# zhengyk19/vit-rpe-rope

Hardware: AMD Instinct MI355X
Metric: train images/sec, CIFAR-10 ViT d=192 L=6 H=6 (higher is better)
Workload: dtype bf16; 1 GPU; CIFAR-10-shaped 32x32 patch4 ViT d=192 L=6 H=6, --pos_encoding rope-axial theta=100, bf16, full train step (fwd+CE+bwd+AdamW), random-init weights; per_gpu_batch=512, global_batch=512, parallelism=dp1, hip_graph=True

## Files before the change

vit-rpe-rope_amd/csrc/misc.hip:

```cpp
#include "common.h"
#include "augment.h"

namespace vitpe {

template <typename T>
__global__ void unfold_kernel(const float* __restrict__ img, T* __restrict__ patches, int B, int Cc, int S, int p) {
  const int g = S / p, P = g * g, Kp = Cc * p * p;
  const long long total = (long long)B * P * Cc * p;
  for (long long idx = (long long)blockIdx.x * blockDim.x + threadIdx.x; idx < total;
       idx += (long long)gridDim.x * blockDim.x) {
    const int ky = (int)(idx % p);
    long long t = idx / p;
    const int ch = (int)(t % Cc); t /= Cc;
    const int n = (int)(t % P);
    const int b = (int)(t / P);
    const int gy = n / g, gx = n % g;
    const float* src = img + (((size_t)b * Cc + ch) * S + gy * p + ky) * S + gx * p;
    T* dst = patches + ((size_t)b * P + n) * Kp + ch * p * p + ky * p;
    for (int kx = 0; kx < p; ++kx) dst[kx] = from_f32<T>(src[kx]);
  }
}

__global__ void unfold8_kernel(const float* __restrict__ img, bf16* __restrict__ patches, int B, int Cc, int S, int p) {
  const int g = S / p, P = g * g, Kp = Cc * p * p, p8 = p / 8;
// ... 365 lines not shown
}

template <typename T, int KD, bool WLDS>
__global__ __launch_bounds__(256) void head_step_kernel(const T* __restrict__ x, const float* __restrict__ gamma,
                                                        const float* __restrict__ beta, const float* __restrict__ Wh,
                                                        const float* __restrict__ bh, const long long* __restrict__ labels,
                                                        float* __restrict__ logits, float* __restrict__ dlogits,
                                                        float* __restrict__ ws_xhat, float* __restrict__ ws_yn,
                                                        float* __restrict__ ws_dyn, T* __restrict__ dx,
                                                        float* __restrict__ per_image, const float* __restrict__ ctl,
                                                        int B, int Ntok, int D, int Cn, float eps) {
  constexpr int HS_LDS = 16 * 768;
  __shared__ float sWh[WLDS ? HS_LDS : 4];
  const int lane = threadIdx.x & 63, wave = threadIdx.x >> 6;
  const int b_raw = blockIdx.x * 4 + wave;
  const bool live = b_raw < B;
  const int b = live ? b_raw : B - 1;
  const float invD = 1.0f / (float)D;
  const float gscale = ctl[0], lscale = ctl[1];
  const int nvalid = min(B, (int)ctl[2]);
  const T* row = x + (size_t)b * Ntok * D;
  float xv[KD], gam[KD], bet[KD];
  float s = 0.f;
#pragma unroll
  for (int k = 0; k < KD; ++k) {
    const int d = lane + 64 * k;
    const bool ok = d < D;
    xv[k] = ok ? to_f32(row[d]) : 0.f;
    gam[k] = ok ? gamma[d] : 0.f;
    bet[k] = ok ? beta[d] : 0.f;
  }
  if (WLDS)
    for (int i = threadIdx.x; i < Cn * D; i += 256) sWh[i] = Wh[i];
  __syncthreads();
  if (!live) return;
#pragma unroll
  for (int k = 0; k < KD; ++k) s += xv[k];
  const float mean = wave_sum(s) * invD;
  float s2 = 0.f;
#pragma unroll
  for (int k = 0; k < KD; ++k) { const float t = (lane + 64 * k < D) ? xv[k] - mean : 0.f; s2 += t * t; }
  const float rstd = 1.0f / sqrtf(wave_sum(s2) * invD + eps);
  float xh[KD], yn[KD];
#pragma unroll
  for (int k = 0; k < KD; ++k) {
    const int d = lane + 64 * k;
    xh[k] = (d < D) ? (xv[k] - mean) * rstd : 0.f;
    yn[k] = xh[k] * gam[k] + bet[k];
    if (d < D) { ws_xhat[(size_t)b * D + d] = xh[k]; ws_yn[(size_t)b * D + d] = yn[k]; }
  }
  float z = -3.0e38f;
  for (int c0 = 0; c0 < Cn; c0 += 8) {
    float part[8];
#pragma unroll
    for (int j = 0; j < 8; ++j) {
      part[j] = 0.f;
      const int cI = min(c0 + j, Cn - 1);
#pragma unroll
      for (int k = 0; k < KD; ++k) {
        const int d = lane + 64 * k;
        part[j] += (d < D) ? yn[k] * (WLDS ? sWh[cI * D + d] : Wh[(size_t)cI * D + d]) : 0.f;
      }
    }
#pragma unroll
    for (int o = 32; o >= 1; o >>= 1)
#pragma unroll
      for (int j = 0; j < 8; ++j) part[j] += __shfl_xor(part[j], o, 64);
#pragma unroll
    for (int j = 0; j < 8; ++j)
      if (lane == c0 + j && c0 + j < Cn) z = part[j] + bh[c0 + j];
  }
  if (lane < Cn) logits[(size_t)b * Cn + lane] = z;
  float m = z;
#pragma unroll
  for (int o = 32; o >= 1; o >>= 1) m = fmaxf(m, __shfl_xor(m, o, 64));
  int am = (lane < Cn && z == m) ? lane : 1 << 20;
#pragma unroll
  for (int o = 32; o >= 1; o >>= 1) am = min(am, __shfl_xor(am, o, 64));
  const float e = lane < Cn ? expf(z - m) : 0.f;
  const float se = wave_sum(e);
  const int y = (int)labels[b];
  const float zy = __shfl(z, y, 64);
  const bool valid = b < nvalid;
  const float dl = (lane < Cn && valid) ? (e * (1.0f / se) - (lane == y ? 1.f : 0.f)) * gscale : 0.f;
  if (lane < Cn) dlogits[(size_t)b * Cn + lane] = dl;
  float dyn[KD];
#pragma unroll
  for (int k = 0; k < KD; ++k) dyn[k] = 0.f;
  for (int c = 0; c < Cn; ++c) {
    const float dc = __shfl(dl, c, 64);
#pragma unroll
    for (int k = 0; k < KD; ++k) {
      const int d = lane + 64 * k;
      dyn[k] += (d < D) ? dc * (WLDS ? sWh[c * D + d] : Wh[(size_t)c * D + d]) : 0.f;
    }
  }
  float t1 = 0.f, t2 = 0.f;
#pragma unroll
  for (int k = 0; k < KD; ++k) {
    const int d = lane + 64 * k;
    if (d < D) ws_dyn[(size_t)b * D + d] = dyn[k];
    const float gv = dyn[k] * gam[k];
    t1 += gv;
    t2 += gv * xh[k];
  }
  t1 = wave_sum(t1) * invD;
  t2 = wave_sum(t2) * invD;
  T* drow = dx + (size_t)b * Ntok * D;
#pragma unroll
  for (int k = 0; k < KD; ++k) {
    const int d = lane + 64 * k;
    if (d < D) drow[d] = from_f32<T>(rstd * (dyn[k] * gam[k] - t1 - xh[k] * t2));
  }
  if (lane == 0) {
    per_image[2 * b] = valid ? ((m + logf(se)) - zy) * lscale : 0.f;
    per_image[2 * b + 1] = (valid && am == y) ? 1.f : 0.f;
  }
}

template <typename T>
__global__ __launch_bounds__(256) void head_bwd_rows_kernel(const float* __restrict__ dlogits, const float* __restrict__ Wh,
                                                            const float* __restrict__ gamma, const float* __restrict__ ws_xhat,
                                                            const float* __restrict__ ws_rstd, float* __restrict__ ws_dyn,
                                                            T* __restrict__ dx, int B, int Ntok, int D, int Cn) {
  const int lane = threadIdx.x & 63, wave = threadIdx.x >> 6;
  const float invD = 1.0f / (float)D;
  for (int b = blockIdx.x * 4 + wave; b < B; b += gridDim.x * 4) {
    float s1 = 0.f, s2 = 0.f;
    for (int d = lane; d < D; d += 64) {
      float dyn = 0.f;
      for (int k = 0; k < Cn; ++k) dyn += dlogits[(size_t)b * Cn + k] * Wh[(size_t)k * D + d];
      ws_dyn[(size_t)b * D + d] = dyn;
      const float gv = dyn * gamma[d];
      s1 += gv;
      s2 += gv * ws_xhat[(size_t)b * D + d];
    }
    s1 = wave_sum(s1) * invD;
    s2 = wave_sum(s2) * invD;
    const float rstd = ws_rstd[b];
    T* drow = dx + (size_t)b * Ntok * D;
    for (int d = lane; d < D; d += 64) {
      const float gv = ws_dyn[(size_t)b * D + d] * gamma[d];
      drow[d] = from_f32<T>(rstd * (gv - s1 - ws_xhat[(size_t)b * D + d] * s2));
    }
    if (D % CH<T>::n == 0) {
      const Chunk16 z16 = {0u, 0u, 0u, 0u};
      for (size_t q = D / CH<T>::n + lane; q < (size_t)Ntok * D / CH<T>::n; q += 64)
        *reinterpret_cast<Chunk16*>(drow + q * CH<T>::n) = z16;
    } else {
      for (size_t q = D + lane; q < (size_t)Ntok * D; q += 64) drow[q] = from_f32<T>(0.f);
    }
  }
}
__global__ void head_bwd_params_kernel(const float* __restrict__ dlogits, const float* __restrict__ ws_yn,
                                       const float* __restrict__ ws_dyn, const float* __restrict__ ws_xhat,
                                       float* dWh, float* dbh, float* dgamma, float* dbeta, int B, int D, int Cn,
                                       int bchunk, const float* __restrict__ per_image, float* out2, float* metric_acc,
                                       float* hp_tick) {
  if (hp_tick != nullptr && blockIdx.x == 0 && blockIdx.y == 0 && threadIdx.x == 0) {
    const float step = hp_tick[5] + 1.0f;
    hp_tick[5] = step;
    hp_tick[6] = 1.0f - powf(hp_tick[1], step);
    hp_tick[7] = 1.0f - powf(hp_tick[2], step);
  }
  if (per_image != nullptr && blockIdx.x == 0 && blockIdx.y == 0) {
    __shared__ float sl[256], sc[256];
    float l = 0.f, cr = 0.f;
    for (int b = threadIdx.x; b < B; b += 256) { l += per_image[2 * b]; cr += per_image[2 * b + 1]; }
    sl[threadIdx.x] = l;
    sc[threadIdx.x] = cr;
    __syncthreads();
    for (int o = 128; o >= 1; o >>= 1) {
      if (threadIdx.x < o) { sl[threadIdx.x] += sl[threadIdx.x + o]; sc[threadIdx.x] += sc[threadIdx.x + o]; }
      __syncthreads();
    }
    if (threadIdx.x == 0) {
      out2[0] = sl[0]; out2[1] = sc[0];
      if (metric_acc != nullptr) { metric_acc[0] += sl[0]; metric_acc[1] += sc[0]; }
    }
  }
  const int idx = blockIdx.x * blockDim.x + threadIdx.x;
  const int b0 = blockIdx.y * bchunk, b1 = min(B, b0 + bchunk);
  const int nW = Cn * D;
  if (idx < nW) {
    const int k = idx / D, d = idx % D;
    float s = 0.f;
    for (int b = b0; b < b1; ++b) s += dlogits[(size_t)b * Cn + k] * ws_yn[(size_t)b * D + d];
    atomicAdd(dWh + idx, s);
  } else if (idx < nW + Cn) {
    const int k = idx - nW;
    float s = 0.f;
    for (int b = b0; b < b1; ++b) s += dlogits[(size_t)b * Cn + k];
    atomicAdd(dbh + k, s);
  } else if (idx < nW + Cn + D) {
    const int d = idx - nW - Cn;
    float sg = 0.f, sb = 0.f;
    for (int b = b0; b < b1; ++b) {
      const float dy = ws_dyn[(size_t)b * D + d];
      sg += dy * ws_xhat[(size_t)b * D + d];
      sb += dy;
    }
    atomicAdd(dgamma + d, sg);
    atomicAdd(dbeta + d, sb);
  }
}

template <typename T>
__global__ void embed_bwd_kernel(const T* __restrict__ dtok, float* dcls, float* dape, T* __restrict__ dpatch,
                                 int B, int Ntok, int D, int bchunk) {
  const int idx = blockIdx.x * blockDim.x + threadIdx.x;
  if (idx >= Ntok * D) return;
  const int n = idx / D, d = idx % D;
  const int b0 = blockIdx.y * bchunk, b1 = min(B, b0 + bchunk);
  float s = 0.f;
  for (int b = b0; b < b1; ++b) {
    const T v = dtok[((size_t)b * Ntok + n) * D + d];
    s += to_f32(v);
    if (n >= 1) dpatch[((size_t)b * (Ntok - 1) + n - 1) * D + d] = v;
  }
  if (n == 0) atomicAdd(dcls + d, s);
  else if (dape) atomicAdd(dape + (size_t)(n - 1) * D + d, s);
}

__global__ void adamw_tick_kernel(float* hp) {
  const float step = hp[5] + 1.0f;
  hp[5] = step;
  hp[6] = 1.0f - powf(hp[1], step);
  hp[7] = 1.0f - powf(hp[2], step);
}
template <int GS>
__global__ void adamw_kernel(float* __restrict__ p, float* __restrict__ g, float* __restrict__ m, float* __restrict__ v,
                             bf16* __restrict__ shadow, const float* __restrict__ hp, long long n, int zero_grad) {
  const float lr = hp[0], b1 = hp[1], b2 = hp[2], eps = hp[3], wd = hp[4], bc1 = hp[6], bc2 = hp[7], gs = hp[GS];
  const float inv_sqrt_bc2 = 1.0f / sqrtf(bc2), step_size = lr / bc1;
  for (long long i = (long long)blockIdx.x * blockDim.x + threadIdx.x; i < n; i += (long long)gridDim.x * blockDim.x) {
    const float gi = g[i] * gs;
    float pi = p[i] * (1.0f - lr * wd);
    const float mi = b1 * m[i] + (1.0f - b1) * gi;
    const float vi = b2 * v[i] + (1.0f - b2) * gi * gi;
    pi -= step_size * mi / (sqrtf(vi) * inv_sqrt_bc2 + eps);
    p[i] = pi; m[i] = mi; v[i] = vi;
    if (shadow) shadow[i] = (bf16)pi;
    if (zero_grad) g[i] = 0.f;
  }
}

static inline int grad_clip_blocks(long long n) { return (int)min((n + 4095) / 4096, (long long)1024); }

__global__ __launch_bounds__(256) void grad_sqnorm_kernel(const float* __restrict__ g, long long n,
                                                          float* __restrict__ partial) {
  const long long head = min(n, (long long)((4 - (int)(((unsigned long long)g >> 2) & 3)) & 3));
  const float4* __restrict__ body = reinterpret_cast<const float4*>(g + head);
  const long long nvec = (n - head) >> 2;
  const long long stride = (long long)gridDim.x * 256;
  float c0 = 0.f, c1 = 0.f, c2 = 0.f, c3 = 0.f;
#define VITPE_SQ_ACC(q) do { c0 = fmaf(q.x, q.x, c0); c1 = fmaf(q.y, q.y, c1); c2 = fmaf(q.z, q.z, c2); c3 = fmaf(q.w, q.w, c3); } while (0)
  long long i = (long long)blockIdx.x * 256 + threadIdx.x;
  for (; i + 3 * stride < nvec; i += 4 * stride) {
    const float4 q0 = body[i], q1 = body[i + stride], q2 = body[i + 2 * stride], q3 = body[i + 3 * stride];
    VITPE_SQ_ACC(q0); VITPE_SQ_ACC(q1); VITPE_SQ_ACC(q2); VITPE_SQ_ACC(q3);
  }
  for (; i < nvec; i += stride) {
    const float4 q = body[i];
    VITPE_SQ_ACC(q);
  }
#undef VITPE_SQ_ACC
  if (blockIdx.x == 0) {
    const long long tail0 = head + 4 * nvec;
    const int t = threadIdx.x;
    if (t < head) c0 = fmaf(g[t], g[t], c0);
    if (t >= 64 && tail0 + (t - 64) < n) c0 = fmaf(g[tail0 + (t - 64)], g[tail0 + (t - 64)], c0);
  }
  float s = (c0 + c1) + (c2 + c3);
#pragma unroll
  for (int o = 32; o >= 1; o >>= 1) s += __shfl_xor(s, o, 64);
  __shared__ float ws[4];
  if ((threadIdx.x & 63) == 0) ws[threadIdx.x >> 6] = s;
  __syncthreads();
  if (threadIdx.x == 0) partial[blockIdx.x] = (ws[0] + ws[1]) + (ws[2] + ws[3]);
}
__global__ __launch_bounds__(64) void grad_clip_finalize_kernel(const float* __restrict__ partial, int nb, float* hp) {
  double s = 0.0;
  for (int i = threadIdx.x; i < nb; i += 64) s += (double)partial[i];
#pragma unroll
  for (int o = 32; o >= 1; o >>= 1) s += __shfl_xor(s, o, 64);
  if (threadIdx.x == 0) {
    const float gs = hp[8];
    const float norm = (float)((double)gs * sqrt(s));
    double coef = (double)hp[12] / ((double)norm + 1e-6);
    coef = coef > 1.0 ? 1.0 : coef;
    const float cf = nb == 0 ? 1.0f : (float)coef;
    hp[10] = norm;
    hp[11] = cf;
    hp[9] = gs * cf;
  }
}
template <typename T>
__global__ void cast_kernel(const float* __restrict__ src, T* __restrict__ dst, long long n) {
  for (long long i = (long long)blockIdx.x * blockDim.x + threadIdx.x; i < n; i += (long long)gridDim.x * blockDim.x)
    dst[i] = from_f32<T>(src[i]);
}
template <typename T>
__global__ void transpose_cast_kernel(const float* __restrict__ src, T* __restrict__ dst, int R, int Cc) {
  __shared__ float tile[32][33];
  const int r0 = blockIdx.y * 32, c0 = blockIdx.x * 32;
  for (int i = threadIdx.y; i < 32; i += 8) {
    const int r = r0 + i, c = c0 + threadIdx.x;
    tile[i][threadIdx.x] = (r < R && c < Cc) ? src[(size_t)r * Cc + c] : 0.f;
  }
  __syncthreads();
  for (int i = threadIdx.y; i < 32; i += 8) {
    const int c = c0 + i, r = r0 + threadIdx.x;
    if (c < Cc && r < R) dst[(size_t)c * R + r] = from_f32<T>(tile[threadIdx.x][i]);
  }
}

struct ShadowDesc { long long src_off, dst_off, dst_off2; int R, C, tile0, kind, HD, kind2, HD2, pad; };

template <typename T>
__global__ __launch_bounds__(256) void refresh_shadows_kernel(const float* __restrict__ flat, T* __restrict__ dst_base,
                                                              const ShadowDesc* __restrict__ desc, int ndesc,
                                                              const unsigned short* __restrict__ tile_map) {
  __shared__ float tile[32][33];
  int d = 0;
  if (tile_map != nullptr) {
    d = tile_map[blockIdx.x];
  } else {
    for (int i = 1; i < ndesc; ++i)
      if ((int)blockIdx.x >= desc[i].tile0) d = i;
  }
  const ShadowDesc ds = desc[d];
  const int t = blockIdx.x - ds.tile0;
  const int tc = (ds.C + 31) / 32;
  const int r0 = (t / tc) * 32, c0 = (t % tc) * 32;
  const float* src = flat + ds.src_off;
  const int tx = threadIdx.x & 31, ty = threadIdx.x >> 5;
  for (int i = ty; i < 32; i += 8) {
    const int r = r0 + i, c = c0 + tx;
    tile[i][tx] = (r < ds.R && c < ds.C) ? src[(size_t)r * ds.C + c] : 0.f;
  }
  __syncthreads();
  auto emit = [&](int kind, T* dst, int hd) {
    if (kind == 0) {
      for (int i = ty; i < 32; i += 8) {
        const int c = c0 + i, r = r0 + tx;
        if (c < ds.C && r < ds.R) dst[(size_t)c * ds.R + r] = from_f32<T>(tile[tx][i]);
      }
    } else if (kind == 6) {
      const int D = ds.C, S = D / 16;
      const float qs = 1.4426950408889634f * rsqrtf((float)hd);
      for (int i = ty; i < 32; i += 8) {
        const int r = r0 + i, c = c0 + tx;
        if (r < ds.R && c < ds.C) {
          const int mat = r / D, rr = r % D, h = rr / 32, f = rr % 32;
          const int sidx = c / 16, hh = (c % 16) / 8, e = c % 8;
          const size_t blk = ((size_t)(h * 3 + mat) * S + sidx);
          dst[(blk * 64 + f + 32 * hh) * 8 + e] = from_f32<T>(tile[i][tx] * (mat == 0 ? qs : 1.0f));
        }
      }
    } else if (kind >= 2) {
      const bool tr = kind >= 4, phi = (kind & 1) != 0;
      const int PR = tr ? ds.C : ds.R;
      const int p0 = tr ? c0 : r0, k0 = tr ? r0 : c0;
      const int kch = hd, KSC = kch / 32, NTr = PR / 16;
      const int kc = k0 / kch, ks = (k0 % kch) / 32;
      const int dd = threadIdx.x * 4, frag = dd >> 9, within = dd & 511, l = within >> 3, e0 = within & 7;
      const int nt = p0 / 16 + frag, cc = l & 15, g = l >> 4;
      if (16 * nt < PR) {
        float v[4];
#pragma unroll
        for (int j = 0; j < 4; ++j) {
          const int e = e0 + j;
          const int k = phi ? (e < 4 ? 4 * g + e : 16 + 4 * g + e - 4) : 8 * g + e;
          v[j] = tr ? tile[k][16 * frag + cc] : tile[16 * frag + cc][k];
        }
        const size_t blk = ((size_t)kc * NTr + nt) * KSC + ks;
        st4(dst + blk * 512 + within, v[0], v[1], v[2], v[3]);
      }
    } else {
      const int D = ds.C, HD = hd, NT = HD / 16, KS = D / 32;
      for (int i = ty; i < 32; i += 8) {
        const int r = r0 + i, c = c0 + tx;
        if (r < ds.R && c < ds.C) {
          const int mat = r / D, rr = r % D, h = rr / HD, nt = (rr % HD) / 16, cc = rr % 16;
          const int ks = c / 32, g = (c % 32) / 8, e = c % 8;
          const size_t blk = (((size_t)(h * 3 + mat) * NT + nt) * KS + ks);
          dst[(blk * 64 + 16 * g + cc) * 8 + e] = from_f32<T>(tile[i][tx]);
        }
      }
    }
  };
  emit(ds.kind, dst_base + ds.dst_off, ds.HD);
  if (ds.kind2 >= 0) emit(ds.kind2, dst_base + ds.dst_off2, ds.HD2);
}

template <typename T>
__global__ void selftest_mma_kernel(const T* __restrict__ A, const T* __restrict__ Bt, const T* __restrict__ Brow,
                                    float* __restrict__ C_row, float* __restrict__ C_tr) {
  __shared__ __attribute__((aligned(16))) T sB[32 * 24];
  const int lane = threadIdx.x, c = lane & 15, g = lane >> 4;
  for (int q = lane; q < 32 * 16; q += 64) sB[(q / 16) * 24 + (q % 16)] = Brow[q];
  __syncthreads();
  f32x4 acc = {0.f, 0.f, 0.f, 0.f};
  mma(ld_frag(A + c * 32 + 8 * g), ld_frag(Bt + c * 32 + 8 * g), acc);
  for (int r = 0; r < 4; ++r) C_row[(4 * g + r) * 16 + c] = acc[r];
  f32x4 acc2 = {0.f, 0.f, 0.f, 0.f};
  mma(ld_frag(A + c * 32 + 8 * g), ld_frag_tr(sB, 24, 8 * g, 8 * g + 4, 0), acc2);
  for (int r = 0; r < 4; ++r) C_tr[(4 * g + r) * 16 + c] = acc2[r];
}

}

using namespace vitpe;

#define GRID1D(n) dim3((unsigned)(((n) + 255) / 256)), dim3(256)

extern "C" int vitpe_unfold(int dtype, const float* img, void* patches, int B, int C, int S, int p, hipStream_t st) {
  VITPE_REQUIRE(img && patches && B >= 0 && C > 0 && p > 0 && S % p == 0 && (dtype == 0 || dtype == 1));
  const long long total = (long long)B * (S / p) * (S / p) * C * p;
  if (total == 0) return 0;
  const unsigned blocks = (unsigned)min((total + 255) / 256, (long long)8192);
  if (dtype == 1 && p % 8 == 0) {
    const long long total8 = total * (p / 8);
    hipLaunchKernelGGL(unfold8_kernel, dim3((unsigned)min((total8 + 255) / 256, (long long)16384)), dim3(256), 0, st, img,
                       (bf16*)patches, B, C, S, p);
    VITPE_CHECK_LAUNCH();
  }
  if (dtype == 1) hipLaunchKernelGGL(unfold_kernel<bf16>, dim3(blocks), dim3(256), 0, st, img, (bf16*)patches, B, C, S, p);
  else hipLaunchKernelGGL(unfold_kernel<float>, dim3(blocks), dim3(256), 0, st, img, (float*)patches, B, C, S, p);
  VITPE_CHECK_LAUNCH();
}

static int launch_unfold_u8(int dtype, const unsigned char* data, const long long* index, const float* mean,
                            const float* stdv, void* patches, float* img_out, int B, int C, int S, int p,
                            const unsigned long long* rng, int pad, int hflip, hipStream_t st) {
  VITPE_REQUIRE(data && mean && stdv && patches && B >= 0 && C > 0 && p > 0 && S % p == 0 && (dtype == 0 || dtype == 1));
  VITPE_REQUIRE(rng == nullptr || (pad >= 0 && pad <= S));
  const long long total = (long long)B * (S / p) * (S / p) * C * p;
  if (total == 0) return 0;
  const unsigned blocks = (unsigned)min((total + 255) / 256, (long long)8192);
  if (rng != nullptr) {
    if (dtype == 1)
      hipLaunchKernelGGL((unfold_u8_kernel<bf16, true>), dim3(blocks), dim3(256), 0, st, data, index, mean, stdv, (bf16*)patches, img_out, B, C, S, p, rng, pad, hflip);
    else
      hipLaunchKernelGGL((unfold_u8_kernel<float, true>), dim3(blocks), dim3(256), 0, st, data, index, mean, stdv, (float*)patches, img_out, B, C, S, p, rng, pad, hflip);
  } else {
    if (dtype == 1)
      hipLaunchKernelGGL((unfold_u8_kernel<bf16, false>), dim3(blocks), dim3(256), 0, st, data, index, mean, stdv, (bf16*)patches, img_out, B, C, S, p, rng, 0, 0);
    else
      hipLaunchKernelGGL((unfold_u8_kernel<float, false>), dim3(blocks), dim3(256), 0, st, data, index, mean, stdv, (float*)patches, img_out, B, C, S, p, rng, 0, 0);
  }
  VITPE_CHECK_LAUNCH();
}

extern "C" int vitpe_unfold_u8(int dtype, const unsigned char* data, const long long* index, const float* mean,
                               const float* stdv, void* patches, float* img_out, int B, int C, int S, int p,
                               hipStream_t st) {
  return launch_unfold_u8(dtype, data, index, mean, stdv, patches, img_out, B, C, S, p, nullptr, 0, 0, st);
}

extern "C" int vitpe_unfold_u8_aug(int dtype, const unsigned char* data, const long long* index, const float* mean,
                                   const float* stdv, void* patches, float* img_out, int B, int C, int S, int p,
                                   const unsigned long long* rng, int pad, int hflip, hipStream_t st) {
  return launch_unfold_u8(dtype, data, index, mean, stdv, patches, img_out, B, C, S, p, rng, pad, hflip, st);
}

extern "C" int vitpe_augment_params(const unsigned long long* rng, int* out, int B, int pad, int hflip, hipStream_t st) {
  VITPE_REQUIRE(rng && B >= 0 && (out || B == 0) && pad >= 0);
  if (B == 0) return 0;
  hipLaunchKernelGGL(augment_params_kernel, GRID1D(B), 0, st, rng, out, B, pad, hflip);
  VITPE_CHECK_LAUNCH();
}

extern "C" int vitpe_relative_position_index(long long* out, int L, hipStream_t st) {
  VITPE_REQUIRE(out && L > 0);
  hipLaunchKernelGGL(rel_index_kernel, GRID1D(L * L), 0, st, out, L);
  VITPE_CHECK_LAUNCH();
}
extern "C" int vitpe_l1_distance_matrix(long long* out, int G, hipStream_t st) {
  VITPE_REQUIRE(out && G > 0);
  hipLaunchKernelGGL(l1_matrix_kernel, GRID1D(G * G * G * G), 0, st, out, G);
  VITPE_CHECK_LAUNCH();
}
extern "C" int vitpe_rope_axial_tables(const float* inv_freq, float* cosv, float* sinv, int G, int half, hipStream_t st) {
  VITPE_REQUIRE(inv_freq && cosv && sinv && G > 0 && half > 0 && half % 2 == 0);
  hipLaunchKernelGGL(rope_axial_kernel, GRID1D(G * G * half), 0, st, inv_freq, cosv, sinv, G, half);
  VITPE_CHECK_LAUNCH();
}
extern "C" int vitpe_rope_mixed_tables(const float* freqs, float* cosv, float* sinv, int H, int G, int half, hipStream_t st) {
  VITPE_REQUIRE(freqs && cosv && sinv && H > 0 && G > 0 && half > 0);
  hipLaunchKernelGGL(rope_mixed_kernel, GRID1D(H * G * G * half), 0, st, freqs, cosv, sinv, H, G, half);
  VITPE_CHECK_LAUNCH();
}
extern "C" int vitpe_relative_bias(const float* table, float* out, int H, int L, hipStream_t st) {
  VITPE_REQUIRE(table && out && H > 0 && L > 0);
  hipLaunchKernelGGL(rel_bias_kernel, GRID1D(H * L * L), 0, st, table, out, H, L);
  VITPE_CHECK_LAUNCH();
}
extern "C" int vitpe_polynomial_bias(const float* coeff, float* out, int H, int G, int degree, int per_head, hipStream_t st) {
  VITPE_REQUIRE(coeff && out && H > 0 && G > 0 && degree >= 0);
  const int L = G * G + 1;
  hipLaunchKernelGGL(poly_bias_kernel, GRID1D(H * L * L), 0, st, coeff, out, H, G, degree, per_head);
  VITPE_CHECK_LAUNCH();
}
extern "C" int vitpe_relative_bias_bwd(const float* dbias, float* dtable, int H, int L, hipStream_t st) {
  VITPE_REQUIRE(dbias && dtable && H > 0 && L > 0);
  hipLaunchKernelGGL(rel_bias_bwd_kernel, GRID1D(H * (2 * L - 1)), 0, st, dbias, dtable, H, L);
  VITPE_CHECK_LAUNCH();
}
extern "C" int vitpe_polynomial_bias_bwd(const float* dbias, float* dcoeff, int H, int G, int degree, int per_head,
                                         hipStream_t st) {
  VITPE_REQUIRE(dbias && dcoeff && H > 0 && G > 0 && degree >= 0);
  hipLaunchKernelGGL(poly_bias_bwd_kernel, dim3((per_head ? H : 1) * (degree + 1)), dim3(256), 0, st, dbias, dcoeff, H, G,
                     degree, per_head);
  VITPE_CHECK_LAUNCH();
}
extern "C" int vitpe_rope_mixed_tables_bwd(const float* freqs, const float* dcos, const float* dsin, float* dfreqs, int H,
                                           int G, int half, hipStream_t st) {
  VITPE_REQUIRE(freqs && dcos && dsin && dfreqs && H > 0 && G > 0 && half > 0);
  hipLaunchKernelGGL(rope_mixed_bwd_kernel, GRID1D(2 * H * half), 0, st, freqs, dcos, dsin, dfreqs, H, G, half);
  VITPE_CHECK_LAUNCH();
}
extern "C" int vitpe_apply_rotary(const float* x, float* y, const float* cosv, const float* sinv, int B, int H, int P,
                                  int HD, int per_head, hipStream_t st) {
  VITPE_REQUIRE(x && y && cosv && sinv && B >= 0 && H > 0 && P > 0 && HD > 0 && HD % 2 == 0);
  const long long total = (long long)B * H * P * (HD / 2);
  if (total == 0) return 0;
  hipLaunchKernelGGL(rotary_kernel, GRID1D(total), 0, st, x, y, cosv, sinv, total, H, P, HD / 2, per_head);
  VITPE_CHECK_LAUNCH();
}

extern "C" int vitpe_head_fwd(int dtype, const void* x, const float* gamma, const float* beta, const float* Wh,
                              const float* bh, float* logits, float* ws_xhat, float* ws_yn, float* ws_rstd, int B,
                              int Ntok, int D, int Cn, float eps, hipStream_t st) {
  VITPE_REQUIRE(x && gamma && beta && Wh && bh && logits && B >= 0 && (dtype == 0 || dtype == 1));
  VITPE_REQUIRE((ws_xhat == nullptr) == (ws_yn == nullptr) && (ws_xhat == nullptr) == (ws_rstd == nullptr));
  if (B == 0) return 0;
  const int blocks = min((B + 3) / 4, 1024);
  if (dtype == 1)
    hipLaunchKernelGGL(head_fwd_kernel<bf16>, dim3(blocks), dim3(256), 0, st, (const bf16*)x, gamma, beta, Wh, bh,
                       logits, ws_xhat, ws_yn, ws_rstd, B, Ntok, D, Cn, eps);
  else
    hipLaunchKernelGGL(head_fwd_kernel<float>, dim3(blocks), dim3(256), 0, st, (const float*)x, gamma, beta, Wh, bh,
                       logits, ws_xhat, ws_yn, ws_rstd, B, Ntok, D, Cn, eps);
  VITPE_CHECK_LAUNCH();
}
extern "C" int vitpe_cross_entropy(const float* logits, const long long* labels, float* dlogits, float* out2, int B,
                                   int Cn, float grad_scale, hipStream_t st) {
  VITPE_REQUIRE(logits && labels && out2 && B > 0 && Cn > 0);
  hipLaunchKernelGGL(ce_kernel, dim3(1), dim3(256), 0, st, logits, labels, dlogits, out2, B, Cn, grad_scale,
                     (const float*)nullptr, (float*)nullptr);
  VITPE_CHECK_LAUNCH();
}
extern "C" int vitpe_cross_entropy_ctl(const float* logits, const long long* labels, float* dlogits, float* out2,
                                       float* metric_acc, const float* ctl, int B, int Cn, hipStream_t st) {
  VITPE_REQUIRE(logits && labels && out2 && ctl && B > 0 && Cn > 0);
  hipLaunchKernelGGL(ce_kernel, dim3(1), dim3(256), 0, st, logits, labels, dlogits, out2, B, Cn, 0.f, ctl, metric_acc);
  VITPE_CHECK_LAUNCH();
}
extern "C" int vitpe_head_bwd(int dtype, const float* dlogits, const float* Wh, const float* gamma,
                              const float* ws_xhat, const float* ws_yn, const float* ws_rstd, float* ws_dyn, void* dx,
                              float* dWh, float* dbh, float* dgamma, float* dbeta, int B, int Ntok, int D, int Cn,
                              hipStream_t st) {
  VITPE_REQUIRE(dlogits && Wh && gamma && ws_xhat && ws_yn && ws_rstd && ws_dyn && dx && dWh && dbh && dgamma && dbeta);
  VITPE_REQUIRE(B >= 0 && (dtype == 0 || dtype == 1));
  if (B == 0) return 0;
  const int blocks = min((B + 3) / 4, 1024);
  if (dtype == 1)
    hipLaunchKernelGGL(head_bwd_rows_kernel<bf16>, dim3(blocks), dim3(256), 0, st, dlogits, Wh, gamma, ws_xhat,
                       ws_rstd, ws_dyn, (bf16*)dx, B, Ntok, D, Cn);
  else
    hipLaunchKernelGGL(head_bwd_rows_kernel<float>, dim3(blocks), dim3(256), 0, st, dlogits, Wh, gamma, ws_xhat,
                       ws_rstd, ws_dyn, (float*)dx, B, Ntok, D, Cn);
  int e = (int)hipGetLastError();
  if (e) return e;
  hipLaunchKernelGGL(head_bwd_params_kernel, dim3((Cn * D + Cn + D + 255) / 256, (B + 31) / 32), dim3(256), 0, st,
                     dlogits, ws_yn, ws_dyn, ws_xhat, dWh, dbh, dgamma, dbeta, B, D, Cn, 32, (const float*)nullptr, (float*)nullptr, (float*)nullptr,
                     (float*)nullptr);
  VITPE_CHECK_LAUNCH();
}
extern "C" int vitpe_head_loss(int dtype, const void* x, const float* gamma, const float* beta, const float* Wh,
                               const float* bh, const long long* labels, float* logits, float* dlogits, float* ws_xhat,
                               float* ws_yn, float* ws_dyn, void* dx, float* out2, float* metric_acc, float* scratch,
                               float* dWh, float* dbh, float* dgamma, float* dbeta, int B, int Ntok, int D, int Cn,
                               float eps, float grad_scale, hipStream_t st) {
  VITPE_REQUIRE(x && gamma && beta && Wh && bh && labels && logits && dlogits && ws_xhat && ws_yn && ws_dyn && dx && out2 &&
                scratch && dWh && dbh && dgamma && dbeta && B >= 0 && (dtype == 0 || dtype == 1));
  if (Cn < 1 || Cn > 64) return (int)hipErrorNotSupported;
  if (B == 0) return 0;
  const int blocks = min((B + 3) / 4, 1024);
  if (dtype == 1)
    hipLaunchKernelGGL(head_loss_kernel<bf16>, dim3(blocks), dim3(256), 0, st, (const bf16*)x, gamma, beta, Wh, bh, labels,
                       logits, dlogits, ws_xhat, ws_yn, ws_dyn, (bf16*)dx, out2, metric_acc, scratch, B, Ntok, D, Cn, eps,
                       grad_scale);
  else
    hipLaunchKernelGGL(head_loss_kernel<float>, dim3(blocks), dim3(256), 0, st, (const float*)x, gamma, beta, Wh, bh, labels,
                       logits, dlogits, ws_xhat, ws_yn, ws_dyn, (float*)dx, out2, metric_acc, scratch, B, Ntok, D, Cn, eps,
                       grad_scale);
  int e = (int)hipGetLastError();
  if (e) return e;
  hipLaunchKernelGGL(head_bwd_params_kernel, dim3((Cn * D + Cn + D + 255) / 256, (B + 31) / 32), dim3(256), 0, st,
                     dlogits, ws_yn, ws_dyn, ws_xhat, dWh, dbh, dgamma, dbeta, B, D, Cn, 32, (const float*)nullptr, (float*)nullptr, (float*)nullptr,
                     (float*)nullptr);
  VITPE_CHECK_LAUNCH();
}
template <typename T>
static int head_step_launch(const T* x, const float* gamma, const float* beta, const float* Wh, const float* bh,
                            const long long* labels, float* logits, float* dlogits, float* ws_xhat, float* ws_yn,
                            float* ws_dyn, T* dx, float* per_image, const float* ctl, int B, int Ntok, int D, int Cn,
                            float eps, hipStream_t st) {
  const dim3 grid((B + 3) / 4), block(256);
#define VITPE_HEAD_STEP(KD)                                                                                              \
  do {                                                                                                                   \
    if (Cn * D <= 16 * 768)                                                                                              \
      hipLaunchKernelGGL((head_step_kernel<T, KD, true>), grid, block, 0, st, x, gamma, beta, Wh, bh, labels, logits,    \
                         dlogits, ws_xhat, ws_yn, ws_dyn, dx, per_image, ctl, B, Ntok, D, Cn, eps);                      \
    else                                                                                                                 \
      hipLaunchKernelGGL((head_step_kernel<T, KD, false>), grid, block, 0, st, x, gamma, beta, Wh, bh, labels, logits,   \
                         dlogits, ws_xhat, ws_yn, ws_dyn, dx, per_image, ctl, B, Ntok, D, Cn, eps);                      \
  } while (0)
  const int kd = (D + 63) / 64;
  if (kd <= 2) VITPE_HEAD_STEP(2);
  else if (kd == 3) VITPE_HEAD_STEP(3);
  else if (kd <= 6) VITPE_HEAD_STEP(6);
  else if (kd <= 12) VITPE_HEAD_STEP(12);
  else return (int)hipErrorNotSupported;
#undef VITPE_HEAD_STEP
  return (int)hipGetLastError();
}
extern "C" int vitpe_head_step(int dtype, const void* x, const float* gamma, const float* beta, const float* Wh,
                               const float* bh, const long long* labels, float* logits, float* dlogits, float* ws_xhat,
                               float* ws_yn, float* ws_dyn, void* dx, float* out2, float* metric_acc, float* per_image,
                               const float* ctl, float* dWh, float* dbh, float* dgamma, float* dbeta, int B, int Ntok,
                               int D, int Cn, float eps, float* hp_tick, hipStream_t st) {
  VITPE_REQUIRE(x && gamma && beta && Wh && bh && labels && logits && dlogits && ws_xhat && ws_yn && ws_dyn && dx && out2 &&
                per_image && ctl && dWh && dbh && dgamma && dbeta && B >= 0 && (dtype == 0 || dtype == 1));
  if (Cn < 1 || Cn > 64 || D > 768) return (int)hipErrorNotSupported;
  if (B == 0) return 0;
  int e = dtype == 1 ? head_step_launch<bf16>((const bf16*)x, gamma, beta, Wh, bh, labels, logits, dlogits, ws_xhat, ws_yn,
                                              ws_dyn, (bf16*)dx, per_image, ctl, B, Ntok, D, Cn, eps, st)
                     : head_step_launch<float>((const float*)x, gamma, beta, Wh, bh, labels, logits, dlogits, ws_xhat, ws_yn,
                                               ws_dyn, (float*)dx, per_image, ctl, B, Ntok, D, Cn, eps, st);
  if (e) return e;
  hipLaunchKernelGGL(head_bwd_params_kernel, dim3((Cn * D + Cn + D + 255) / 256, (B + 31) / 32), dim3(256), 0, st,
                     dlogits, ws_yn, ws_dyn, ws_xhat, dWh, dbh, dgamma, dbeta, B, D, Cn, 32, (const float*)per_image, out2,
                     metric_acc, hp_tick);
  VITPE_CHECK_LAUNCH();
}
extern "C" int vitpe_embed_bwd(int dtype, const void* dtok, float* dcls, float* dape, void* dpatch, int B, int Ntok,
                               int D, hipStream_t st) {
  VITPE_REQUIRE(dtok && dcls && dpatch && B >= 0 && (dtype == 0 || dtype == 1));
  if (dtype == 1)
    hipLaunchKernelGGL(embed_bwd_kernel<bf16>, dim3((Ntok * D + 255) / 256, (B + 15) / 16), dim3(256), 0, st,
                       (const bf16*)dtok, dcls, dape, (bf16*)dpatch, B, Ntok, D, 16);
  else
    hipLaunchKernelGGL(embed_bwd_kernel<float>, dim3((Ntok * D + 255) / 256, (B + 15) / 16), dim3(256), 0, st,
                       (const float*)dtok, dcls, dape, (float*)dpatch, B, Ntok, D, 16);
  VITPE_CHECK_LAUNCH();
}

extern "C" int vitpe_adamw_step(float* p, float* g, float* m, float* v, void* shadow_bf16, float* hp, long long n,
                                int zero_grad, hipStream_t st) {
  VITPE_REQUIRE(p && g && m && v && hp && n >= 0);
  if (!(zero_grad & 2)) hipLaunchKernelGGL(adamw_tick_kernel, dim3(1), dim3(1), 0, st, hp);
  if (n > 0) {
    const unsigned blocks = (unsigned)min((n + 255) / 256, (long long)4096);
    if (zero_grad & 4)
      hipLaunchKernelGGL(adamw_kernel<9>, dim3(blocks), dim3(256), 0, st, p, g, m, v, (bf16*)shadow_bf16, hp, n, zero_grad & 1);
    else
      hipLaunchKernelGGL(adamw_kernel<8>, dim3(blocks), dim3(256), 0, st, p, g, m, v, (bf16*)shadow_bf16, hp, n, zero_grad & 1);
  }
  VITPE_CHECK_LAUNCH();
}
extern "C" int vitpe_grad_clip_blocks(long long n) { return n > 0 ? grad_clip_blocks(n) : 0; }
extern "C" int vitpe_grad_clip(const float* g, long long n, float* hp, float* partial, int n_partial, hipStream_t st) {
  VITPE_REQUIRE(hp && n >= 0 && (n == 0 || (g && partial)) && ((unsigned long long)g & 3) == 0);
  const int nb = n > 0 ? grad_clip_blocks(n) : 0;
  VITPE_REQUIRE(n_partial >= nb);
  if (nb > 0) hipLaunchKernelGGL(grad_sqnorm_kernel, dim3(nb), dim3(256), 0, st, g, n, partial);
  hipLaunchKernelGGL(grad_clip_finalize_kernel, dim3(1), dim3(64), 0, st, (const float*)partial, nb, hp);
  VITPE_CHECK_LAUNCH();
}
extern "C" int vitpe_cast(int dtype, const float* src, void* dst, long long n, hipStream_t st) {
  VITPE_REQUIRE(src && dst && n >= 0 && (dtype == 0 || dtype == 1));
  if (n == 0) return 0;
  const unsigned blocks = (unsigned)min((n + 255) / 256, (long long)4096);
  if (dtype == 1) hipLaunchKernelGGL(cast_kernel<bf16>, dim3(blocks), dim3(256), 0, st, src, (bf16*)dst, n);
  else hipLaunchKernelGGL(cast_kernel<float>, dim3(blocks), dim3(256), 0, st, src, (float*)dst, n);
  VITPE_CHECK_LAUNCH();
}
extern "C" int vitpe_transpose_cast(int dtype, const float* src, void* dst, int R, int C, hipStream_t st) {
  VITPE_REQUIRE(src && dst && R > 0 && C > 0 && (dtype == 0 || dtype == 1));
  dim3 grid((C + 31) / 32, (R + 31) / 32), block(32, 8);
  if (dtype == 1) hipLaunchKernelGGL(transpose_cast_kernel<bf16>, grid, block, 0, st, src, (bf16*)dst, R, C);
  else hipLaunchKernelGGL(transpose_cast_kernel<float>, grid, block, 0, st, src, (float*)dst, R, C);
  VITPE_CHECK_LAUNCH();
}

extern "C" int vitpe_refresh_shadows(int dtype, const float* flat, void* dst_base, const void* desc, int ndesc,
                                     int total_tiles, const unsigned short* tile_map, hipStream_t st) {
  VITPE_REQUIRE(flat && dst_base && desc && ndesc > 0 && total_tiles > 0 && (dtype == 0 || dtype == 1));
  if (dtype == 1)
    hipLaunchKernelGGL(refresh_shadows_kernel<bf16>, dim3(total_tiles), dim3(256), 0, st, flat, (bf16*)dst_base,
                       (const ShadowDesc*)desc, ndesc, tile_map);
  else
    hipLaunchKernelGGL(refresh_shadows_kernel<float>, dim3(total_tiles), dim3(256), 0, st, flat, (float*)dst_base,
                       (const ShadowDesc*)desc, ndesc, tile_map);
  VITPE_CHECK_LAUNCH();
}

extern "C" int vitpe_selftest_mma(int dtype, const void* A, const void* Bt, const void* Brow, float* C_row, float* C_tr,
                                  hipStream_t st) {
  VITPE_REQUIRE(A && Bt && Brow && C_row && C_tr && (dtype == 0 || dtype == 1));
  if (dtype == 1)
    hipLaunchKernelGGL(selftest_mma_kernel<bf16>, dim3(1), dim3(64), 0, st, (const bf16*)A, (const bf16*)Bt,
                       (const bf16*)Brow, C_row, C_tr);
  else
    hipLaunchKernelGGL(selftest_mma_kernel<float>, dim3(1), dim3(64), 0, st, (const float*)A, (const float*)Bt,
                       (const float*)Brow, C_row, C_tr);
  VITPE_CHECK_LAUNCH();
}

template <int DEPTH>
__global__ __launch_bounds__(256) void read_bw_kernel(const uint4* __restrict__ src, long long nvec, unsigned* sink) {
  const long long stride = (long long)gridDim.x * 256;
  unsigned acc = 0;
  for (long long i = (long long)blockIdx.x * 256 + threadIdx.x; i < nvec; i += stride * DEPTH) {
    uint4 v[DEPTH];
#pragma unroll
    for (int d = 0; d < DEPTH; ++d) v[d] = (i + d * stride < nvec) ? src[i + d * stride] : make_uint4(0, 0, 0, 0);
#pragma unroll
    for (int d = 0; d < DEPTH; ++d) acc ^= v[d].x ^ v[d].y ^ v[d].z ^ v[d].w;
  }
  if (acc == 0x9E3779B9u) *sink = acc;
}
extern "C" int vitpe_debug_read_bw(const void* src, long long bytes, int depth, int workgroups, unsigned* sink, hipStream_t st) {
  VITPE_REQUIRE(src && sink && bytes >= 16 && workgroups > 0 && (depth == 1 || depth == 4 || depth == 8));
  const long long nvec = bytes / 16;
  if (depth == 1) hipLaunchKernelGGL(read_bw_kernel<1>, dim3(workgroups), dim3(256), 0, st, (const uint4*)src, nvec, sink);
  else if (depth == 4) hipLaunchKernelGGL(read_bw_kernel<4>, dim3(workgroups), dim3(256), 0, st, (const uint4*)src, nvec, sink);
  else hipLaunchKernelGGL(read_bw_kernel<8>, dim3(workgroups), dim3(256), 0, st, (const uint4*)src, nvec, sink);
  VITPE_CHECK_LAUNCH();
}

extern "C" int vitpe_abi_version(void) { return 4; }
```

Before: 365,300 images/sec.

## Vectorize head-param, embed backward and shadow-refresh kernels with block-level reductions

Rewrites the head parameter-gradient kernel to use float4 loads, 8-row per-wave accumulation and a shared-memory cross-wave reduction before atomics. The loss and step-tick work moves to a dedicated extra block. Adds a vectorized embed backward kernel that copies 16-byte chunks and reduces rows in LDS before atomics. The shadow refresh gains a whole-tile fast path with 4-wide stores for the QKV layouts. The aim is fewer scalar memory transactions and far fewer atomic operations, at the cost of more code paths and alignment checks.

```diff
diff --git a/vit-rpe-rope_amd/csrc/misc.hip b/vit-rpe-rope_amd/csrc/misc.hip
--- a/vit-rpe-rope_amd/csrc/misc.hip
+++ b/vit-rpe-rope_amd/csrc/misc.hip
@@ -541,57 +541,136 @@
     }
   }
 }
-__global__ void head_bwd_params_kernel(const float* __restrict__ dlogits, const float* __restrict__ ws_yn,
-                                       const float* __restrict__ ws_dyn, const float* __restrict__ ws_xhat,
-                                       float* dWh, float* dbh, float* dgamma, float* dbeta, int B, int D, int Cn,
-                                       int bchunk, const float* __restrict__ per_image, float* out2, float* metric_acc,
-                                       float* hp_tick) {
-  if (hp_tick != nullptr && blockIdx.x == 0 && blockIdx.y == 0 && threadIdx.x == 0) {
-    const float step = hp_tick[5] + 1.0f;
-    hp_tick[5] = step;
-    hp_tick[6] = 1.0f - powf(hp_tick[1], step);
-    hp_tick[7] = 1.0f - powf(hp_tick[2], step);
-  }
-  if (per_image != nullptr && blockIdx.x == 0 && blockIdx.y == 0) {
-    __shared__ float sl[256], sc[256];
-    float l = 0.f, cr = 0.f;
-    for (int b = threadIdx.x; b < B; b += 256) { l += per_image[2 * b]; cr += per_image[2 * b + 1]; }
-    sl[threadIdx.x] = l;
-    sc[threadIdx.x] = cr;
-    __syncthreads();
-    for (int o = 128; o >= 1; o >>= 1) {
-      if (threadIdx.x < o) { sl[threadIdx.x] += sl[threadIdx.x + o]; sc[threadIdx.x] += sc[threadIdx.x + o]; }
+constexpr int HBP_ROWS = 8;
+template <int V> VITPE_DEV void hbp_load(const float* p, float* o);
+template <> VITPE_DEV void hbp_load<4>(const float* p, float* o) {
+  const float4 t = *reinterpret_cast<const float4*>(p);
+  o[0] = t.x; o[1] = t.y; o[2] = t.z; o[3] = t.w;
+}
+template <> VITPE_DEV void hbp_load<1>(const float* p, float* o) { o[0] = *p; }
+
+template <int V>
+__global__ __launch_bounds__(256) void head_bwd_params_kernel(const float* __restrict__ dlogits,
+                                                              const float* __restrict__ ws_yn,
+                                                              const float* __restrict__ ws_dyn,
+                                                              const float* __restrict__ ws_xhat, float* dWh, float* dbh,
+                                                              float* dgamma, float* dbeta, int B, int D, int Cn, int nx,
+                                                              int ny, const float* __restrict__ per_image, float* out2,
+                                                              float* metric_acc, float* hp_tick) {
+  __shared__ float red[2][4][64 * V];
+  if ((int)blockIdx.x == nx * ny) {
+    if (hp_tick != nullptr && threadIdx.x == 0) {
+      const float step = hp_tick[5] + 1.0f;
+      hp_tick[5] = step;
+      hp_tick[6] = 1.0f - powf(hp_tick[1], step);
+      hp_tick[7] = 1.0f - powf(hp_tick[2], step);
+    }
+    if (per_image != nullptr) {
+      float* sl = &red[0][0][0];
+      float* sc = &red[1][0][0];
+      float l = 0.f, cr = 0.f;
+      for (int b = threadIdx.x; b < B; b += 256) { l += per_image[2 * b]; cr += per_image[2 * b + 1]; }
+      sl[threadIdx.x] = l;
+      sc[threadIdx.x] = cr;
       __syncthreads();
-    }
-    if (threadIdx.x == 0) {
-      out2[0] = sl[0]; out2[1] = sc[0];
-      if (metric_acc != nullptr) { metric_acc[0] += sl[0]; metric_acc[1] += sc[0]; }
-    }
-  }
-  const int idx = blockIdx.x * blockDim.x + threadIdx.x;
-  const int b0 = blockIdx.y * bchunk, b1 = min(B, b0 + bchunk);
-  const int nW = Cn * D;
-  if (idx < nW) {
-    const int k = idx / D, d = idx % D;
-    float s = 0.f;
-    for (int b = b0; b < b1; ++b) s += dlogits[(size_t)b * Cn + k] * ws_yn[(size_t)b * D + d];
-    atomicAdd(dWh + idx, s);
-  } else if (idx < nW + Cn) {
-    const int k = idx - nW;
-    float s = 0.f;
-    for (int b = b0; b < b1; ++b) s += dlogits[(size_t)b * Cn + k];
-    atomicAdd(dbh + k, s);
-  } else if (idx < nW + Cn + D) {
-    const int d = idx - nW - Cn;
-    float sg = 0.f, sb = 0.f;
-    for (int b = b0; b < b1; ++b) {
-      const float dy = ws_dyn[(size_t)b * D + d];
-      sg += dy * ws_xhat[(size_t)b * D + d];
-      sb += dy;
-    }
-    atomicAdd(dgamma + d, sg);
-    atomicAdd(dbeta + d, sb);
-  }
+      if (threadIdx.x < 128) { l += sl[threadIdx.x + 128]; cr += sc[threadIdx.x + 128]; }
+      __syncthreads();
+      if (threadIdx.x < 128) { sl[threadIdx.x] = l; sc[threadIdx.x] = cr; }
+      __syncthreads();
+      if (threadIdx.x < 64) {
+        l += sl[threadIdx.x + 64];
+        cr += sc[threadIdx.x + 64];
+#pragma unroll
+        for (int o = 32; o >= 1; o >>= 1) { l += __shfl_down(l, o, 64); cr += __shfl_down(cr, o, 64); }
+        if (threadIdx.x == 0) {
+          out2[0] = l; out2[1] = cr;
+          if (metric_acc != nullptr) { metric_acc[0] += l; metric_acc[1] += cr; }
+        }
+      }
+    }
+    return;
+  }
+  const int lane = threadIdx.x & 63, wave = threadIdx.x >> 6;
+  const int bx = blockIdx.x % nx, by = blockIdx.x / nx;
+  const int DV = D / V, nW = Cn * DV, nG = nW + DV, nitems = nG + (Cn + V - 1) / V;
+  const int item = bx * 64 + lane;
+  const int b0 = by * (4 * HBP_ROWS) + wave * HBP_ROWS;
+  float sa[V], sb[V];
+#pragma unroll
+  for (int e = 0; e < V; ++e) sa[e] = sb[e] = 0.f;
+  if (item < nW) {
+    const int k = item / DV, d = (item % DV) * V;
+    float w[HBP_ROWS], y[HBP_ROWS][V];
+#pragma unroll
+    for (int j = 0; j < HBP_ROWS; ++j) {
+      const int b = min(b0 + j, B - 1);
+      w[j] = dlogits[(size_t)b * Cn + k];
+      hbp_load<V>(ws_yn + (size_t)b * D + d, y[j]);
+    }
+#pragma unroll
+    for (int j = 0; j < HBP_ROWS; ++j)
+      if (b0 + j < B) {
+#pragma unroll
+        for (int e = 0; e < V; ++e) sa[e] += w[j] * y[j][e];
+      }
+  } else if (item < nG) {
+    const int d = (item - nW) * V;
+    float dy[HBP_ROWS][V], xh[HBP_ROWS][V];
+#pragma unroll
+    for (int j = 0; j < HBP_ROWS; ++j) {
+      const int b = min(b0 + j, B - 1);
+      hbp_load<V>(ws_dyn + (size_t)b * D + d, dy[j]);
+      hbp_load<V>(ws_xhat + (size_t)b * D + d, xh[j]);
+    }
+#pragma unroll
+    for (int j = 0; j < HBP_ROWS; ++j)
+      if (b0 + j < B) {
+#pragma unroll
+        for (int e = 0; e < V; ++e) { sa[e] += dy[j][e] * xh[j][e]; sb[e] += dy[j][e]; }
+      }
+  } else if (item < nitems) {
+    const int k0 = (item - nG) * V;
+    float w[HBP_ROWS][V];
+#pragma unroll
+    for (int j = 0; j < HBP_ROWS; ++j)
+#pragma unroll
+      for (int e = 0; e < V; ++e) w[j][e] = (b0 + j < B && k0 + e < Cn) ? dlogits[(size_t)(b0 + j) * Cn + k0 + e] : 0.f;
+#pragma unroll
+    for (int j = 0; j < HBP_ROWS; ++j)
+#pragma unroll
+      for (int e = 0; e < V; ++e) sa[e] += w[j][e];
+  }
+#pragma unroll
+  for (int e = 0; e < V; ++e) { red[0][wave][lane * V + e] = sa[e]; red[1][wave][lane * V + e] = sb[e]; }
+  __syncthreads();
+  if ((int)threadIdx.x < 64 * V) {
+    const int i = threadIdx.x, it = bx * 64 + i / V, e = i % V;
+    const float ta = (red[0][0][i] + red[0][1][i]) + (red[0][2][i] + red[0][3][i]);
+    if (it < nW) {
+      atomicAdd(dWh + (size_t)it * V + e, ta);
+    } else if (it < nG) {
+      atomicAdd(dgamma + (it - nW) * V + e, ta);
+      atomicAdd(dbeta + (it - nW) * V + e, (red[1][0][i] + red[1][1][i]) + (red[1][2][i] + red[1][3][i]));
+    } else if (it < nitems && (it - nG) * V + e < Cn) {
+      atomicAdd(dbh + (it - nG) * V + e, ta);
+    }
+  }
+}
+static inline bool aligned16(const void* p) { return ((unsigned long long)p & 15) == 0; }
+static void head_bwd_params_launch(const float* dlogits, const float* ws_yn, const float* ws_dyn, const float* ws_xhat,
+                                   float* dWh, float* dbh, float* dgamma, float* dbeta, int B, int D, int Cn,
+                                   const float* per_image, float* out2, float* metric_acc, float* hp_tick, hipStream_t st) {
+  const bool vec = D % 4 == 0 && aligned16(ws_yn) && aligned16(ws_dyn) && aligned16(ws_xhat);
+  const int V = vec ? 4 : 1;
+  const int nitems = Cn * (D / V) + D / V + (Cn + V - 1) / V;
+  const int nx = (nitems + 63) / 64, ny = (B + 4 * HBP_ROWS - 1) / (4 * HBP_ROWS);
+  const dim3 grid(nx * ny + ((per_image != nullptr || hp_tick != nullptr) ? 1 : 0));
+  if (vec)
+    hipLaunchKernelGGL(head_bwd_params_kernel<4>, grid, dim3(256), 0, st, dlogits, ws_yn, ws_dyn, ws_xhat, dWh, dbh, dgamma,
+                       dbeta, B, D, Cn, nx, ny, per_image, out2, metric_acc, hp_tick);
+  else
+    hipLaunchKernelGGL(head_bwd_params_kernel<1>, grid, dim3(256), 0, st, dlogits, ws_yn, ws_dyn, ws_xhat, dWh, dbh, dgamma,
+                       dbeta, B, D, Cn, nx, ny, per_image, out2, metric_acc, hp_tick);
 }
 
 template <typename T>
@@ -609,6 +688,52 @@
   }
   if (n == 0) atomicAdd(dcls + d, s);
   else if (dape) atomicAdd(dape + (size_t)(n - 1) * D + d, s);
+}
+constexpr int EB_ROWS = 8;
+template <typename T>
+__global__ __launch_bounds__(256, 4) void embed_bwd_vec_kernel(const T* __restrict__ dtok, float* dcls, float* dape,
+                                                            T* __restrict__ dpatch, int B, int Ntok, int D) {
+  constexpr int E = CH<T>::n;
+  __shared__ float red[4][64 * E];
+  const int lane = threadIdx.x & 63, wave = threadIdx.x >> 6;
+  const int rowlen = Ntok * D;
+  const int f = (blockIdx.x * 64 + lane) * E;
+  const bool okq = f < rowlen;
+  const int n = okq ? f / D : 0, d = okq ? f % D : 0;
+  const int b0 = blockIdx.y * (4 * EB_ROWS) + wave * EB_ROWS;
+  Chunk16 v[EB_ROWS];
+#pragma unroll
+  for (int j = 0; j < EB_ROWS; ++j) {
+    v[j] = Chunk16{0u, 0u, 0u, 0u};
+    if (okq && b0 + j < B) v[j] = *reinterpret_cast<const Chunk16*>(dtok + (size_t)(b0 + j) * rowlen + f);
+  }
+  if (okq && n >= 1) {
+#pragma unroll
+    for (int j = 0; j < EB_ROWS; ++j)
+      if (b0 + j < B)
+        *reinterpret_cast<Chunk16*>(dpatch + ((size_t)(b0 + j) * (Ntok - 1) + n - 1) * D + d) = v[j];
+  }
+  float s[E];
+#pragma unroll
+  for (int e = 0; e < E; ++e) s[e] = 0.f;
+#pragma unroll
+  for (int j = 0; j < EB_ROWS; ++j) {
+    float t[E];
+    chunk_to_f32<T>(v[j], t);
+#pragma unroll
+    for (int e = 0; e < E; ++e) s[e] += t[e];
+  }
+#pragma unroll
+  for (int e = 0; e < E; ++e) red[wave][lane * E + e] = s[e];
+  __syncthreads();
+  for (int i = threadIdx.x; i < 64 * E; i += 256) {
+    const int g = blockIdx.x * 64 * E + i;
+    if (g < rowlen) {
+      const float t = (red[0][i] + red[1][i]) + (red[2][i] + red[3][i]);
+      if (g < D) atomicAdd(dcls + g, t);
+      else if (dape) atomicAdd(dape + (g - D), t);
+    }
+  }
 }
 
 __global__ void adamw_tick_kernel(float* hp) {
@@ -719,16 +844,18 @@
       if ((int)blockIdx.x >= desc[i].tile0) d = i;
   }
   const ShadowDesc ds = desc[d];
+  const int tx = threadIdx.x & 31, ty = threadIdx.x >> 5;
   const int t = blockIdx.x - ds.tile0;
   const int tc = (ds.C + 31) / 32;
   const int r0 = (t / tc) * 32, c0 = (t % tc) * 32;
   const float* src = flat + ds.src_off;
-  const int tx = threadIdx.x & 31, ty = threadIdx.x >> 5;
   for (int i = ty; i < 32; i += 8) {
     const int r = r0 + i, c = c0 + tx;
     tile[i][tx] = (r < ds.R && c < ds.C) ? src[(size_t)r * ds.C + c] : 0.f;
   }
   __syncthreads();
+  const bool whole = ds.R % 32 == 0 && ds.C % 32 == 0;
+  const int dd = threadIdx.x * 4, frag = dd >> 9, within = dd & 511, l = within >> 3, e0 = within & 7;
   auto emit = [&](int kind, T* dst, int hd) {
     if (kind == 0) {
       for (int i = ty; i < 32; i += 8) {
@@ -738,13 +865,21 @@
     } else if (kind == 6) {
       const int D = ds.C, S = D / 16;
       const float qs = 1.4426950408889634f * rsqrtf((float)hd);
-      for (int i = ty; i < 32; i += 8) {
-        const int r = r0 + i, c = c0 + tx;
-        if (r < ds.R && c < ds.C) {
-          const int mat = r / D, rr = r % D, h = rr / 32, f = rr % 32;
-          const int sidx = c / 16, hh = (c % 16) / 8, e = c % 8;
-          const size_t blk = ((size_t)(h * 3 + mat) * S + sidx);
-          dst[(blk * 64 + f + 32 * hh) * 8 + e] = from_f32<T>(tile[i][tx] * (mat == 0 ? qs : 1.0f));
+      if (whole && D % 32 == 0) {
+        const int mat = r0 / D, h = (r0 % D) / 32, f = l & 31, hh = l >> 5;
+        const float sc = mat == 0 ? qs : 1.0f;
+        const size_t blk = ((size_t)(h * 3 + mat) * S + c0 / 16 + frag);
+        const float* sp = &tile[f][16 * frag + 8 * hh + e0];
+        st4(dst + blk * 512 + within, sp[0] * sc, sp[1] * sc, sp[2] * sc, sp[3] * sc);
+      } else {
+        for (int i = ty; i < 32; i += 8) {
+          const int r = r0 + i, c = c0 + tx;
+          if (r < ds.R && c < ds.C) {
+            const int mat = r / D, rr = r % D, h = rr / 32, f = rr % 32;
+            const int sidx = c / 16, hh = (c % 16) / 8, e = c % 8;
+            const size_t blk = ((size_t)(h * 3 + mat) * S + sidx);
+            dst[(blk * 64 + f + 32 * hh) * 8 + e] = from_f32<T>(tile[i][tx] * (mat == 0 ? qs : 1.0f));
+          }
         }
       }
     } else if (kind >= 2) {
@@ -753,28 +888,35 @@
       const int p0 = tr ? c0 : r0, k0 = tr ? r0 : c0;
       const int kch = hd, KSC = kch / 32, NTr = PR / 16;
       const int kc = k0 / kch, ks = (k0 % kch) / 32;
-      const int dd = threadIdx.x * 4, frag = dd >> 9, within = dd & 511, l = within >> 3, e0 = within & 7;
       const int nt = p0 / 16 + frag, cc = l & 15, g = l >> 4;
       if (16 * nt < PR) {
-        float v[4];
+        float w[4];
 #pragma unroll
         for (int j = 0; j < 4; ++j) {
           const int e = e0 + j;
           const int k = phi ? (e < 4 ? 4 * g + e : 16 + 4 * g + e - 4) : 8 * g + e;
-          v[j] = tr ? tile[k][16 * frag + cc] : tile[16 * frag + cc][k];
+          w[j] = tr ? tile[k][16 * frag + cc] : tile[16 * frag + cc][k];
         }
         const size_t blk = ((size_t)kc * NTr + nt) * KSC + ks;
-        st4(dst + blk * 512 + within, v[0], v[1], v[2], v[3]);
+        st4(dst + blk * 512 + within, w[0], w[1], w[2], w[3]);
       }
     } else {
       const int D = ds.C, HD = hd, NT = HD / 16, KS = D / 32;
-      for (int i = ty; i < 32; i += 8) {
-        const int r = r0 + i, c = c0 + tx;
-        if (r < ds.R && c < ds.C) {
-          const int mat = r / D, rr = r % D, h = rr / HD, nt = (rr % HD) / 16, cc = rr % 16;
-          const int ks = c / 32, g = (c % 32) / 8, e = c % 8;
-          const size_t blk = (((size_t)(h * 3 + mat) * NT + nt) * KS + ks);
-          dst[(blk * 64 + 16 * g + cc) * 8 + e] = from_f32<T>(tile[i][tx]);
+      if (whole && HD % 16 == 0) {
+        const int r = r0 + 16 * frag, mat = r / D, rr = r % D, h = rr / HD, nt = (rr % HD) / 16;
+        const int cc = l & 15, g = l >> 4;
+        const size_t blk = (((size_t)(h * 3 + mat) * NT + nt) * KS + c0 / 32);
+        const float* sp = &tile[16 * frag + cc][8 * g + e0];
+        st4(dst + blk * 512 + within, sp[0], sp[1], sp[2], sp[3]);
+      } else {
+        for (int i = ty; i < 32; i += 8) {
+          const int r = r0 + i, c = c0 + tx;
+          if (r < ds.R && c < ds.C) {
+            const int mat = r / D, rr = r % D, h = rr / HD, nt = (rr % HD) / 16, cc = rr % 16;
+            const int ks = c / 32, g = (c % 32) / 8, e = c % 8;
+            const size_t blk = (((size_t)(h * 3 + mat) * NT + nt) * KS + ks);
+            dst[(blk * 64 + 16 * g + cc) * 8 + e] = from_f32<T>(tile[i][tx]);
+          }
         }
       }
     }
@@ -963,9 +1105,7 @@
                        ws_rstd, ws_dyn, (float*)dx, B, Ntok, D, Cn);
   int e = (int)hipGetLastError();
   if (e) return e;
-  hipLaunchKernelGGL(head_bwd_params_kernel, dim3((Cn * D + Cn + D + 255) / 256, (B + 31) / 32), dim3(256), 0, st,
-                     dlogits, ws_yn, ws_dyn, ws_xhat, dWh, dbh, dgamma, dbeta, B, D, Cn, 32, (const float*)nullptr, (float*)nullptr, (float*)nullptr,
-                     (float*)nullptr);
+  head_bwd_params_launch(dlogits, ws_yn, ws_dyn, ws_xhat, dWh, dbh, dgamma, dbeta, B, D, Cn, nullptr, nullptr, nullptr, nullptr, st);
   VITPE_CHECK_LAUNCH();
 }
 extern "C" int vitpe_head_loss(int dtype, const void* x, const float* gamma, const float* beta, const float* Wh,
@@ -988,9 +1128,7 @@
                        grad_scale);
   int e = (int)hipGetLastError();
   if (e) return e;
-  hipLaunchKernelGGL(head_bwd_params_kernel, dim3((Cn * D + Cn + D + 255) / 256, (B + 31) / 32), dim3(256), 0, st,
-                     dlogits, ws_yn, ws_dyn, ws_xhat, dWh, dbh, dgamma, dbeta, B, D, Cn, 32, (const float*)nullptr, (float*)nullptr, (float*)nullptr,
-                     (float*)nullptr);
+  head_bwd_params_launch(dlogits, ws_yn, ws_dyn, ws_xhat, dWh, dbh, dgamma, dbeta, B, D, Cn, nullptr, nullptr, nullptr, nullptr, st);
   VITPE_CHECK_LAUNCH();
 }
 template <typename T>
@@ -1031,14 +1169,25 @@
                      : head_step_launch<float>((const float*)x, gamma, beta, Wh, bh, labels, logits, dlogits, ws_xhat, ws_yn,
                                                ws_dyn, (float*)dx, per_image, ctl, B, Ntok, D, Cn, eps, st);
   if (e) return e;
-  hipLaunchKernelGGL(head_bwd_params_kernel, dim3((Cn * D + Cn + D + 255) / 256, (B + 31) / 32), dim3(256), 0, st,
-                     dlogits, ws_yn, ws_dyn, ws_xhat, dWh, dbh, dgamma, dbeta, B, D, Cn, 32, (const float*)per_image, out2,
-                     metric_acc, hp_tick);
+  head_bwd_params_launch(dlogits, ws_yn, ws_dyn, ws_xhat, dWh, dbh, dgamma, dbeta, B, D, Cn, per_image, out2, metric_acc, hp_tick,
+                         st);
   VITPE_CHECK_LAUNCH();
 }
 extern "C" int vitpe_embed_bwd(int dtype, const void* dtok, float* dcls, float* dape, void* dpatch, int B, int Ntok,
                                int D, hipStream_t st) {
   VITPE_REQUIRE(dtok && dcls && dpatch && B >= 0 && (dtype == 0 || dtype == 1));
+  if (B == 0 || Ntok <= 0 || D <= 0) return 0;
+  const int E = dtype == 1 ? 8 : 4;
+  if (D % E == 0 && aligned16(dtok) && aligned16(dpatch)) {
+    const dim3 grid((Ntok * D / E + 63) / 64, (B + 4 * EB_ROWS - 1) / (4 * EB_ROWS)), block(256);
+    if (dtype == 1)
+      hipLaunchKernelGGL(embed_bwd_vec_kernel<bf16>, grid, block, 0, st, (const bf16*)dtok, dcls, dape, (bf16*)dpatch, B,
+                         Ntok, D);
+    else
+      hipLaunchKernelGGL(embed_bwd_vec_kernel<float>, grid, block, 0, st, (const float*)dtok, dcls, dape, (float*)dpatch, B,
+                         Ntok, D);
+    VITPE_CHECK_LAUNCH();
+  }
   if (dtype == 1)
     hipLaunchKernelGGL(embed_bwd_kernel<bf16>, dim3((Ntok * D + 255) / 256, (B + 15) / 16), dim3(256), 0, st,
                        (const bf16*)dtok, dcls, dape, (bf16*)dpatch, B, Ntok, D, 16);
```

New measurement: 368,600 images/sec, median of 2. No clear change (+0.9%).
